# ueda0319/neddf

Hardware: NVIDIA H100
Metric: ray-samples/s (800x800x192) (higher is better)
Workload: dtype f16x3-split operands, f32 accumulate

## Files before the change

neddf_b200/csrc/field_tc.cu:

```cuda
#include "tc_ptx.cuh"

#include <algorithm>
#include <cstring>

namespace neddf {
namespace tc {

constexpr int kStages = 3;
constexpr int kConsumers = 256;
constexpr int kConsumerWarps = kConsumers / 32;
constexpr int kThreads = kConsumers + 128;
constexpr uint32_t kConsumerRegs = 232, kProducerRegs = 40;

constexpr uint32_t kOffHHi = 0;
constexpr uint32_t kOffHLo = kOffHHi + kHBytes;
constexpr uint32_t kOffAuxHi = kOffHLo + kHBytes;
constexpr uint32_t kOffAuxLo = kOffAuxHi + kAuxBytes;
constexpr uint32_t kOffRing = kOffAuxLo + kAuxBytes;
constexpr uint32_t kOffScratch = kOffRing + kStages * kChunkBytes;

struct Scratch {
  float geo[kTileS][12];
  uint64_t full[kStages];
  uint64_t empty[kStages];
};
constexpr uint32_t kSmemBytes = kOffScratch + sizeof(Scratch);
static_assert(kSmemBytes <= 227 * 1024, "shared memory budget");

constexpr int kGroup = kRows / kTileS;
constexpr uint32_t kParkH = kHBytes / kGroup, kParkAux = kAuxBytes / kGroup;
constexpr uint32_t kParkBytes = 2 * kParkH + 2 * kParkAux;

struct TcLayer {
  int aux_ksteps;
  int h_ksteps;
};

struct TcParams {
  FieldParams f;
  TcLayer layer[kMaxHidden];
  int chunks_per_tile;
  int dist_chunks;
  const unsigned char* w_tc;
  const float* bias;
  int* status;
  int eval;
  int density_only;
  unsigned char* park;
};

__device__ __forceinline__ uint32_t cluster_ctarank() {
  uint32_t r;
  asm volatile("mov.u32 %0, %%cluster_ctarank;" : "=r"(r));
  return r;
}
__device__ __forceinline__ void cluster_sync_all() {
  asm volatile("barrier.cluster.arrive.release.aligned;\nbarrier.cluster.wait.acquire.aligned;" ::: "memory");
}
__device__ __forceinline__ uint32_t mapa_u32(uint32_t saddr, uint32_t rank) {
  uint32_t r;
  asm volatile("mapa.shared::cluster.u32 %0, %1, %2;" : "=r"(r) : "r"(saddr), "r"(rank));
  return r;
}
__device__ __forceinline__ void mbar_arrive_remote(uint32_t caddr) {
  asm volatile("mbarrier.arrive.release.cluster.shared::cluster.b64 _, [%0];" ::"r"(caddr) : "memory");
}
__device__ __forceinline__ void mbar_wait_cluster(uint64_t* bar, uint32_t parity) {
  asm volatile(
      "{\n"
      ".reg .pred p;\n"
      "TC_WAITC:\n"
      "mbarrier.try_wait.parity.acquire.cluster.shared::cta.b64 p, [%0], %1;\n"
      "@p bra TC_DONEC;\n"
      "bra TC_WAITC;\n"
      "TC_DONEC:\n"
      "}\n" ::"r"(smem_u32(bar)),
      "r"(parity)
      : "memory");
}
__device__ __forceinline__ void tma_bulk_g2s_pair(uint32_t dst_smem, const void* src, uint32_t bytes, uint64_t* bar) {
  asm volatile(
      "cp.async.bulk.shared::cluster.global.mbarrier::complete_tx::bytes.multicast::cluster [%0], [%1], %2, [%3], %4;" ::"r"(
          dst_smem),
      "l"(src), "r"(bytes), "r"(smem_u32(bar)), "h"((uint16_t)3)
      : "memory");
}

__device__ __forceinline__ void tile_geometry(const FieldParams& p, float (*geo)[12], int64_t n0, int s, int64_t n_total) {
  const SampleIn in = sample_input(p, n0 + s, n_total);
#pragma unroll
  for (int i = 0; i < 3; ++i) {
    geo[s][i] = in.pos[i];
    geo[s][3 + i] = in.dir[i];
    geo[s][6 + i] = in.var[i];
  }
}

__device__ __forceinline__ void write_pos_embedding(const FieldParams& p, const float (*geo)[12], unsigned char* aux_hi,
                                                    unsigned char* aux_lo, int s, int sub, int nsub, bool scaled,
                                                    float& bad, int rows = 4) {
  const int half = 3 * p.embed_pos;
  for (int idx = sub; idx < half; idx += nsub) {
    int e = idx / 3, d = idx - 3 * e;
    PeEntry q = pe_entry(e, geo[s][d], geo[s][6 + d], p.lowpass[e]);
    float sc_ = scaled ? q.scale_s : q.scale_0;
    float g = q.freq * sc_;
    const float js = g * q.c, jc = -g * q.s;
    store_sample(aux_hi, aux_lo, kAuxK, s, idx, sc_ * q.s, d == 0 ? js : 0.f, d == 1 ? js : 0.f, d == 2 ? js : 0.f, bad, rows);
    store_sample(aux_hi, aux_lo, kAuxK, s, half + idx, sc_ * q.c, d == 0 ? jc : 0.f, d == 1 ? jc : 0.f, d == 2 ? jc : 0.f, bad, rows);
  }
}

__device__ __forceinline__ void bar_consumers() { asm volatile("bar.sync 1, %0;" ::"n"(kConsumers) : "memory"); }

template <bool kLoad>
__device__ __forceinline__ void park_move(unsigned char* smem, unsigned char* slot, int j, int tid) {
#pragma unroll
  for (int b = 0; b < 4; ++b) {
    const uint32_t bytes = b < 2 ? kParkH : kParkAux;
    const uint32_t so = (b == 0 ? kOffHHi : b == 1 ? kOffHLo : b == 2 ? kOffAuxHi : kOffAuxLo) + (uint32_t)j * bytes;
    const uint32_t go = b < 2 ? b * kParkH : 2 * kParkH + (b - 2) * kParkAux;
    uint4* s = reinterpret_cast<uint4*>(smem + so);
    uint4* g = slot ? reinterpret_cast<uint4*>(slot + go) : nullptr;
    constexpr int kIt = kParkH / 16 / kConsumers;
    uint4 v[kIt];
#pragma unroll
    for (int it = 0; it < kIt; ++it) {
      const uint32_t idx = tid + it * kConsumers;
      if (idx < bytes / 16) v[it] = kLoad ? (g ? g[idx] : make_uint4(0u, 0u, 0u, 0u)) : s[idx];
    }
#pragma unroll
    for (int it = 0; it < kIt; ++it) {
      const uint32_t idx = tid + it * kConsumers;
      if (idx < bytes / 16) {
        if (kLoad) s[idx] = v[it];
        else g[idx] = v[it];
      }
    }
  }
}

enum { kPhPrologue, kPhDistance, kPhHeads, kPhColour, kPhPark, kPhTiles, kPhCount };
#ifdef NEDDF_TC_PHASE_CLOCKS
__device__ unsigned long long g_tc_phase[kPhCount];
#define TC_PHASE(i)                        \
  do {                                     \
    if (tid == 0) {                        \
      const long long now_ = clock64();    \
      ph_sum[i] += now_ - ph_t;            \
      ph_t = now_;                         \
    }                                      \
  } while (0)
#else
#define TC_PHASE(i) \
  do {              \
  } while (0)
#endif

template <int ACT, bool PAIR>
__global__ void __launch_bounds__(kThreads, 1) field_tc_kernel(const __grid_constant__ TcParams P) {
  extern __shared__ __align__(1024) unsigned char smem[];
  const FieldParams& p = P.f;
  unsigned char* h_hi = smem + kOffHHi;
  unsigned char* h_lo = smem + kOffHLo;
  unsigned char* aux_hi = smem + kOffAuxHi;
  unsigned char* aux_lo = smem + kOffAuxLo;
  unsigned char* ring = smem + kOffRing;
  Scratch* sc = reinterpret_cast<Scratch*>(smem + kOffScratch);

  const int tid = threadIdx.x;
  const int warp = tid >> 5, lane = tid & 31;
  const int n_hidden = p.n_ddf + p.n_col;

  const int64_t n_total = field_total(p);
  const int64_t n_tiles = (n_total + kTileS - 1) / kTileS;
  const uint32_t rank = PAIR ? cluster_ctarank() : 0;
  const int64_t unit = PAIR ? (int64_t)(blockIdx.x >> 1) : (int64_t)blockIdx.x;
  const int64_t n_units = PAIR ? (int64_t)(gridDim.x >> 1) : (int64_t)gridDim.x;
  const int64_t units_total = PAIR ? (n_tiles + 1) / 2 : n_tiles;
  int64_t my_tiles = 0;
  if (unit < units_total) my_tiles = (units_total - 1 - unit) / n_units + 1;
  auto tile_of = [&](int64_t t) { return PAIR ? 2 * (unit + t * n_units) + rank : unit + t * n_units; };
  const int group = P.eval && !P.density_only ? kGroup : 1;
  const int chunks_end = P.density_only ? P.dist_chunks : P.chunks_per_tile;

  if (tid == 0) {
    for (int i = 0; i < kStages; ++i) {
      mbar_init(&sc->full[i], 1);
      mbar_init(&sc->empty[i], PAIR ? 2 * kConsumerWarps : kConsumerWarps);
    }
    mbar_fence_init();
  }
  __syncthreads();
  if (PAIR) cluster_sync_all();

  if (warp >= kConsumerWarps) {
    asm volatile("setmaxnreg.dec.sync.aligned.u32 %0;" ::"n"(kProducerRegs));
    if (warp == kConsumerWarps && lane == 0) {
      int64_t g = 0;
      auto push = [&](int c) {
        const int s = (int)(g % kStages);
        if (g >= kStages) mbar_wait_cluster(&sc->empty[s], (uint32_t)((g / kStages - 1) & 1));
        mbar_expect_tx(&sc->full[s], kChunkBytes);
        const unsigned char* src = P.w_tc + (size_t)c * kChunkBytes;
        const uint32_t dst = smem_u32(ring + s * kChunkBytes);
        if (PAIR) tma_bulk_g2s_pair(dst + rank * (kChunkBytes / 2), src + rank * (kChunkBytes / 2), kChunkBytes / 2, &sc->full[s]);
        else tma_bulk_g2s(dst, src, kChunkBytes, &sc->full[s]);
        ++g;
      };
      for (int64_t base = 0; base < my_tiles; base += group) {
        const int gn = (int)std::min<int64_t>(group, my_tiles - base);
        for (int i = 0; i < gn; ++i)
          for (int c = 0; c < P.dist_chunks; ++c) push(c);
        for (int c = P.dist_chunks; c < chunks_end; ++c) push(c);
      }
    }
  } else {
    asm volatile("setmaxnreg.inc.sync.aligned.u32 %0;" ::"n"(kConsumerRegs));
    const int wg = tid >> 7;
    const int chb = 128 * wg + 16 * ((tid & 127) >> 5) + (lane >> 2);
    const int cq = 2 * (lane & 3);
    const int hs = tid >> 3, hj = (tid >> 1) & 3, hk = tid & 1;
    const int hbase = lane & ~7;
    float bad = 0.f;
    __half2 badh = __floats2half2_rn(0.f, 0.f);
    uint32_t peer_empty[kStages];
#pragma unroll
    for (int i = 0; i < kStages; ++i) peer_empty[i] = PAIR ? mapa_u32(smem_u32(&sc->empty[i]), rank ^ 1) : 0u;
    auto release = [&](int64_t g) {
      if (lane == 0) {
        const int s = (int)(g % kStages);
        mbar_arrive(&sc->empty[s]);
        if (PAIR) mbar_arrive_remote(peer_empty[s]);
      }
    };
    int64_t g = 0;
    HeadOut head;
    std::memset(&head, 0, sizeof(head));
#ifdef NEDDF_TC_PHASE_CLOCKS
    long long ph_sum[kPhCount] = {}, ph_t = clock64();
#endif

    unsigned char* park = P.park + (size_t)blockIdx.x * kGroup * kParkBytes;

    auto layer = [&](int l, int64_t base, int gn) {
      const int64_t n0 = tile_of(base) * kTileS;
      const TcLayer L = P.layer[l];
      const bool cgroup = P.eval && l >= p.n_ddf;
      float acc[2][64];
#pragma unroll
      for (int i = 0; i < 64; ++i) {
        acc[0][i] = 0.f;
        acc[1][i] = 0.f;
      }
      fence_regs(acc[0]);
      fence_regs(acc[1]);
      const int nk = L.aux_ksteps + L.h_ksteps;
      for (int ks = 0; ks < nk; ++ks, ++g) {
        const int s = (int)(g % kStages);
        mbar_wait(&sc->full[s], (uint32_t)((g / kStages) & 1));
        const uint32_t w = smem_u32(ring + s * kChunkBytes);
        uint64_t bhi, blo;
        if (ks < L.aux_ksteps) {
          bhi = make_desc(smem_u32(aux_hi) + ks * 256, 128, kAuxK * 16);
          blo = make_desc(smem_u32(aux_lo) + ks * 256, 128, kAuxK * 16);
        } else {
          const int kh = ks - L.aux_ksteps;
          bhi = make_desc(smem_u32(h_hi) + kh * 256, 128, kHK * 16);
          blo = make_desc(smem_u32(h_lo) + kh * 256, 128, kHK * 16);
        }
        wgmma_fence();
#pragma unroll
        for (int mb = 0; mb < 2; ++mb) {
          const uint32_t aoff = (uint32_t)(16 * wg + 8 * mb) * 256;
          const uint64_t ahi = make_desc(w + aoff, 128, 256), alo = make_desc(w + kChunkBytes / 2 + aoff, 128, 256);
          wgmma_n128<0, 1>(acc[mb], ahi, bhi, 1);
          wgmma_n128<0, 1>(acc[mb], alo, bhi, 1);
          wgmma_n128<0, 1>(acc[mb], ahi, blo, 1);
        }
        wgmma_commit();
        if (ks > 0) {
          wgmma_wait<1>();
          release(g - 1);
        }
      }
      wgmma_wait<0>();
      fence_regs(acc[0]);
      fence_regs(acc[1]);
      release(g - 1);
      bar_consumers();

      const float* bias = P.bias + (size_t)l * kWidth;
#pragma unroll
      for (int mb = 0; mb < 2; ++mb) {
#pragma unroll
        for (int r = 0; r < 2; ++r) {
          const int ch = chb + 64 * mb + 8 * r;
          const float b = __ldg(bias + ch);
#pragma unroll
          for (int q = 0; q < 4; ++q) {
            float y[2], d1[2];
            const uint32_t off = (uint32_t)(q * (kHK * 16) + ch * 16 + cq * 2);
#pragma unroll
            for (int e = 0; e < 2; ++e) {
              const float xpre = acc[mb][4 * q + 2 * r + e] + b;
              if (p.save_pre) {
                const int64_t n = n0 + 8 * q + cq + e;
                if (n < n_total) {
                  float* dst = p.save_pre + (((size_t)l * p.n + n) * 4) * kWidth + ch;
                  dst[0] = xpre;
#pragma unroll
                  for (int j = 1; j < 4; ++j) dst[j * kWidth] = acc[mb][16 * j + 4 * q + 2 * r + e];
                }
              }
              tc_hidden_act<ACT>(xpre, y[e], d1[e]);
            }
            uint32_t hi, lo;
            split2h(y[0], y[1], hi, lo, badh);
            *reinterpret_cast<uint32_t*>(h_hi + off) = hi;
            *reinterpret_cast<uint32_t*>(h_lo + off) = lo;
            if (cgroup) {
#pragma unroll
              for (int j = 1; j < 4; ++j) {
#pragma unroll
                for (int e = 0; e < 2; ++e) tc_hidden_act<ACT>(acc[mb][16 * j + 4 * q + 2 * r + e] + b, y[e], d1[e]);
                split2h(y[0], y[1], hi, lo, badh);
                *reinterpret_cast<uint32_t*>(h_hi + off + j * 4 * (kHK * 16)) = hi;
                *reinterpret_cast<uint32_t*>(h_lo + off + j * 4 * (kHK * 16)) = lo;
              }
            } else {
#pragma unroll
              for (int j = 1; j < 4; ++j) {
                const float g0 = d1[0] * acc[mb][16 * j + 4 * q + 2 * r];
                const float g1 = d1[1] * acc[mb][16 * j + 4 * q + 2 * r + 1];
                split2h(g0, g1, hi, lo, badh);
                *reinterpret_cast<uint32_t*>(h_hi + off + j * 4 * (kHK * 16)) = hi;
                *reinterpret_cast<uint32_t*>(h_lo + off + j * 4 * (kHK * 16)) = lo;
              }
            }
          }
        }
      }
      bar_consumers();
      TC_PHASE(l < p.n_ddf ? kPhDistance : kPhColour);

      const int hrow = 32 * hj + hs;
      const uint32_t hrow_off = (uint32_t)((hrow >> 3) * (kHK * 16) + (hrow & 7) * 2);
      const int rot = hj + 4 * hk;
      auto hval = [&](int k) {
        return __half2float(*reinterpret_cast<const __half*>(h_hi + hrow_off + k * 16)) +
               __half2float(*reinterpret_cast<const __half*>(h_lo + hrow_off + k * 16));
      };
      if (l == p.n_ddf - 1) {
        float pd = 0.f, pa = 0.f;
#pragma unroll 4
        for (int kk = 0; kk < 128; ++kk) {
          const int k = 128 * hk + ((kk + rot) & 127);
          const float v = hval(k);
          const float2 wv = __ldg(reinterpret_cast<const float2*>(p.w_head_da) + k);
          pd = fmaf(v, wv.x, pd);
          pa = fmaf(v, wv.y, pa);
        }
        pd += __shfl_xor_sync(0xffffffffu, pd, 1);
        pa += __shfl_xor_sync(0xffffffffu, pa, 1);
        float ddf[4], aux[4];
#pragma unroll
        for (int j = 0; j < 4; ++j) {
          ddf[j] = __shfl_sync(0xffffffffu, pd, hbase + 2 * j);
          aux[j] = __shfl_sync(0xffffffffu, pa, hbase + 2 * j);
        }
        const int rows = P.eval ? 1 : 4;
        if (hj == 0 && hk == 0) {
          ddf[0] += __ldg(p.b_head + 0);
          aux[0] += __ldg(p.b_head + 1);
          head_density(ddf, aux, p.d_near, p.aux_grad_scale, p.density_act, head);
          const int kn = p.n_e0 + p.n_d;
          if (!P.density_only) {
#pragma unroll
            for (int c = 0; c < 3; ++c) store_sample(aux_hi, aux_lo, kAuxK, hs, kn + c, head.normal[c], 0.f, 0.f, 0.f, bad, rows);
          }
          const int64_t n = n0 + hs;
          if (n < n_total) {
            int64_t ray_, on;
            int j_;
            field_map(p, n, ray_, j_, on);
            if (p.distance) p.distance[on] = head.distance;
            if (p.density) p.density[on] = head.density;
            if (p.aux_grad) p.aux_grad[on] = head.aux;
          }
        }
        if (!P.density_only) {
          const int s = tid >> 3, sub = tid & 7;
          write_pos_embedding(p, sc->geo, aux_hi, aux_lo, s, sub, 8, false, bad, rows);
          const int dhalf = 3 * p.embed_dir;
          for (int idx = sub; idx < dhalf; idx += 8) {
            int e = idx / 3, d = idx - 3 * e;
            float sn, cs;
            sincosf((float)(1u << e) * sc->geo[s][3 + d], &sn, &cs);
            store_sample(aux_hi, aux_lo, kAuxK, s, p.n_e0 + idx, sn, 0.f, 0.f, 0.f, bad, rows);
            store_sample(aux_hi, aux_lo, kAuxK, s, p.n_e0 + dhalf + idx, cs, 0.f, 0.f, 0.f, bad, rows);
          }
          for (int k = p.n_e0 + p.n_d + 3 + sub; k < kAuxK; k += 8)
            store_sample(aux_hi, aux_lo, kAuxK, s, k, 0.f, 0.f, 0.f, 0.f, bad, rows);
        }
        bar_consumers();
      } else if (l == n_hidden - 1) {
        if (cgroup) {
          const int row = tid >> 1, ck = tid & 1;
          const uint32_t row_off = (uint32_t)((row >> 3) * (kHK * 16) + (row & 7) * 2);
          float pc[3] = {0.f, 0.f, 0.f};
#pragma unroll 4
          for (int kk = 0; kk < 128; ++kk) {
            const int k = 128 * ck + ((kk + 4 * ck) & 127);
            const float v = __half2float(*reinterpret_cast<const __half*>(h_hi + row_off + k * 16)) +
                            __half2float(*reinterpret_cast<const __half*>(h_lo + row_off + k * 16));
            const float4 wv = __ldg(reinterpret_cast<const float4*>(p.w_head_col) + k);
            pc[0] = fmaf(v, wv.x, pc[0]);
            pc[1] = fmaf(v, wv.y, pc[1]);
            pc[2] = fmaf(v, wv.z, pc[2]);
          }
#pragma unroll
          for (int c = 0; c < 3; ++c) pc[c] += __shfl_xor_sync(0xffffffffu, pc[c], 1);
          const int64_t n = tile_of(base + (row >> 5)) * kTileS + (row & 31);
          if (ck == 0 && (row >> 5) < gn && n < n_total && p.color) {
            int64_t ray_, on;
            int j_;
            field_map(p, n, ray_, j_, on);
#pragma unroll
            for (int c = 0; c < 3; ++c) p.color[3 * on + c] = pc[c] + __ldg(p.b_head + 2 + c);
          }
        } else {
          float pc[3] = {0.f, 0.f, 0.f};
#pragma unroll 4
          for (int kk = 0; kk < 128; ++kk) {
            const int k = 128 * hk + ((kk + rot) & 127);
            const float v = hval(k);
            const float4 wv = __ldg(reinterpret_cast<const float4*>(p.w_head_col) + k);
            pc[0] = fmaf(v, wv.x, pc[0]);
            pc[1] = fmaf(v, wv.y, pc[1]);
            pc[2] = fmaf(v, wv.z, pc[2]);
          }
          float colv[4][3];
#pragma unroll
          for (int c = 0; c < 3; ++c) {
            pc[c] += __shfl_xor_sync(0xffffffffu, pc[c], 1);
#pragma unroll
            for (int j = 0; j < 4; ++j) colv[j][c] = __shfl_sync(0xffffffffu, pc[c], hbase + 2 * j);
          }
          const int64_t n = n0 + hs;
          if (hj == 0 && hk == 0 && n < n_total) {
            float col[3], colJ[3][3];
#pragma unroll
            for (int c = 0; c < 3; ++c) {
              col[c] = colv[0][c] + __ldg(p.b_head + 2 + c);
#pragma unroll
              for (int j = 0; j < 3; ++j) colJ[j][c] = colv[1 + j][c];
            }
            int64_t ray_, on;
            int j_;
            field_map(p, n, ray_, j_, on);
            if (p.color) {
              p.color[3 * on + 0] = col[0];
              p.color[3 * on + 1] = col[1];
              p.color[3 * on + 2] = col[2];
            }
            if (p.penalty) p.penalty[on] = field_penalty(head, col, colJ, p.distance_range_max, p.penalty_weight);
          }
        }
      }
      fence_async_smem();
      bar_consumers();
      TC_PHASE(l == p.n_ddf - 1 || l == n_hidden - 1 ? kPhHeads : l < p.n_ddf ? kPhDistance : kPhColour);
    };

    for (int64_t base = 0; base < my_tiles; base += group) {
      const int gn = (int)std::min<int64_t>(group, my_tiles - base);
      for (int gi = 0; gi < gn; ++gi) {
        const int64_t n0 = tile_of(base + gi) * kTileS;
        if (tid < kTileS) tile_geometry(p, sc->geo, n0, tid, n_total);
        bar_consumers();
        {
          const int s = tid >> 3, sub = tid & 7;
          write_pos_embedding(p, sc->geo, aux_hi, aux_lo, s, sub, 8, true, bad);
          for (int k = p.n_e0 + sub; k < 64; k += 8) store_sample(aux_hi, aux_lo, kAuxK, s, k, 0.f, 0.f, 0.f, 0.f, bad);
        }
        fence_async_smem();
        bar_consumers();
        TC_PHASE(kPhPrologue);
#ifdef NEDDF_TC_PHASE_CLOCKS
        if (tid == 0) ++ph_sum[kPhTiles];
#endif
        for (int l = 0; l < p.n_ddf; ++l) layer(l, base + gi, 1);
        if (P.eval && !P.density_only) {
          park_move<false>(smem, park + gi * kParkBytes, 0, tid);
          TC_PHASE(kPhPark);
        }
      }
      if (P.density_only) continue;
      if (P.eval) {
        bar_consumers();
        for (int j = 0; j < kGroup; ++j) park_move<true>(smem, j < gn ? park + j * kParkBytes : nullptr, j, tid);
        fence_async_smem();
        bar_consumers();
        TC_PHASE(kPhPark);
      }
      for (int l = p.n_ddf; l < n_hidden; ++l) layer(l, base, gn);
    }
#ifdef NEDDF_TC_PHASE_CLOCKS
    if (tid == 0)
      for (int i = 0; i < kPhCount; ++i) atomicAdd(&g_tc_phase[i], (unsigned long long)ph_sum[i]);
#endif
    const float2 m = __half22float2(badh);
    if (!(fmaxf(bad, fmaxf(m.x, m.y)) < 65504.0f) && P.status) atomicOr(P.status, 4);
  }
  if (PAIR) cluster_sync_all();
}

struct TcPackArgs {
  const float* w[kMaxHidden];
  const float* b[kMaxHidden];
  int k_in[kMaxHidden];
  int aux_real[kMaxHidden];
  int aux_pad[kMaxHidden];
  int ksteps[kMaxHidden];
  int chunk0[kMaxHidden];
  int n_hidden;
};

__global__ void tc_pack_hidden_kernel(TcPackArgs a, unsigned char* __restrict__ dst, float* __restrict__ bias) {
  const int l = blockIdx.y;
  const int total = a.ksteps[l] * kWidth * 16;
  for (int idx = blockIdx.x * blockDim.x + threadIdx.x; idx < total; idx += gridDim.x * blockDim.x) {
    const int k = idx & 15, m = (idx >> 4) & (kWidth - 1), ks = idx >> 12;
    const int kk = ks * 16 + k;
    int row;
    if (kk < a.aux_pad[l]) row = (kk < a.aux_real[l]) ? kk : -1;
    else row = a.aux_real[l] + (kk - a.aux_pad[l]);
    if (row >= a.k_in[l]) row = -1;
    const float w = (row >= 0) ? a.w[l][(size_t)row * kWidth + m] : 0.f;
    const __half hi = __float2half_rn(w);
    const __half lo = __float2half_rn(w - __half2float(hi));
    unsigned char* chunk = dst + (size_t)(a.chunk0[l] + ks) * kChunkBytes;
    *reinterpret_cast<__half*>(chunk + wchunk_off(m, k)) = hi;
    *reinterpret_cast<__half*>(chunk + kChunkBytes / 2 + wchunk_off(m, k)) = lo;
  }
  if (blockIdx.x == 0)
    for (int c = threadIdx.x; c < kWidth; c += blockDim.x) bias[l * kWidth + c] = a.b[l][c];
}

struct TcStorage {
  unsigned char* d_w = nullptr;
  float* d_bias = nullptr;
  int* d_status = nullptr;
  unsigned char* d_park = nullptr;
  int chunks_per_tile = 0;
  int dist_chunks = 0;
  TcLayer layer[kMaxHidden];
  TcPackArgs pack;
};

template <int N>
__global__ void __launch_bounds__(256, 1) tc_selftest_kernel(const float* __restrict__ A, const float* __restrict__ B, int k,
                                                            float* __restrict__ C) {
  extern __shared__ __align__(1024) unsigned char smem[];
  constexpr int kA = kChunkBytes / 2;
  const int ksteps = k / 16;
  unsigned char* a_buf = smem;
  unsigned char* b_hi = smem + (size_t)ksteps * kA;
  unsigned char* b_lo = b_hi + (size_t)N * k * 2;
  const int tid = threadIdx.x;
  for (int i = tid; i < 128 * k; i += blockDim.x) {
    const int m = i / k, kk = i % k;
    const float v = A[i];
    const __half hi = __float2half_rn(v), lo = __float2half_rn(v - __half2float(hi));
    unsigned char* chunk = a_buf + (size_t)(kk / 16) * kA;
    *reinterpret_cast<__half*>(chunk + wchunk_off(m, kk & 15)) = hi;
    *reinterpret_cast<__half*>(chunk + kA / 2 + wchunk_off(m, kk & 15)) = lo;
  }
  for (int i = tid; i < N * k; i += blockDim.x) {
    const int n = i / k, kk = i % k;
    const float v = B[i];
    const __half hi = __float2half_rn(v), lo = __float2half_rn(v - __half2float(hi));
    *reinterpret_cast<__half*>(b_hi + act_off(n, kk, k)) = hi;
    *reinterpret_cast<__half*>(b_lo + act_off(n, kk, k)) = lo;
  }
  fence_async_smem();
  __syncthreads();
  if (tid < 128 * 2) {
    const int wg = tid >> 7, lane = tid & 31;
    constexpr int R = N / 2;
    float acc[R];
#pragma unroll
    for (int i = 0; i < R; ++i) acc[i] = 0.f;
    fence_regs(acc);
    wgmma_fence();
    for (int ks = 0; ks < ksteps; ++ks) {
      const uint32_t w = smem_u32(a_buf + (size_t)ks * kA) + (uint32_t)(8 * wg) * 256;
      const uint64_t ahi = make_desc(w, 128, 256), alo = make_desc(w + kA / 2, 128, 256);
      const uint64_t bhi = make_desc(smem_u32(b_hi) + ks * 256, 128, k * 16), blo = make_desc(smem_u32(b_lo) + ks * 256, 128, k * 16);
      if constexpr (N == 128) {
        wgmma_n128<0, 1>(acc, ahi, bhi, 1);
        wgmma_n128<0, 1>(acc, alo, bhi, 1);
        wgmma_n128<0, 1>(acc, ahi, blo, 1);
      } else {
        wgmma_n16<0, 1>(acc, ahi, bhi, 1);
        wgmma_n16<0, 1>(acc, alo, bhi, 1);
        wgmma_n16<0, 1>(acc, ahi, blo, 1);
      }
    }
    wgmma_commit();
    wgmma_wait<0>();
    fence_regs(acc);
    const int row = 64 * wg + 16 * ((tid & 127) >> 5) + (lane >> 2);
#pragma unroll
    for (int i = 0; i < R; ++i) {
      const int m = row + 8 * ((i >> 1) & 1), n = 8 * (i >> 2) + 2 * (lane & 3) + (i & 1);
      C[(size_t)m * N + n] = acc[i];
    }
  }
}

}

static bool is_skip_layer(const neddf_field* f, int l) {
  for (int i = 0; i < f->cfg.n_skips; ++i)
    if (f->cfg.skips[i] == l - 1) return true;
  return false;
}

bool tc_supported(const neddf_field* f) {
  const int n_e0 = 6 * f->cfg.embed_pos_rank, off_h = n_e0 + 6 * f->cfg.embed_dir_rank + 3;
  return n_e0 <= 64 && off_h <= tc::kAuxK && f->cfg.ddf_layer_width == kWidth && f->cfg.col_layer_width == kWidth;
}

static int32_t tc_ensure(neddf_field* f) {
  if (f->tc) return NEDDF_OK;
  tc::TcStorage* S = new tc::TcStorage();
  const int n_hidden = f->n_ddf + f->n_col;
  int chunk = 0;
  std::memset(&S->pack, 0, sizeof(S->pack));
  S->pack.n_hidden = n_hidden;
  for (int l = 0; l < n_hidden; ++l) {
    int aux_real = 0, aux_pad = 0, h_k = 0;
    if (l == 0) { aux_real = f->proto.n_e0; aux_pad = 64; }
    else if (l < f->n_ddf) { if (is_skip_layer(f, l)) { aux_real = f->proto.n_e0; aux_pad = 64; } h_k = kWidth; }
    else if (l == f->n_ddf) { aux_real = f->proto.off_h; aux_pad = tc::kAuxK; h_k = kWidth; }
    else h_k = kWidth;
    S->layer[l].aux_ksteps = aux_pad / 16;
    S->layer[l].h_ksteps = h_k / 16;
    S->pack.k_in[l] = f->shape_in[l];
    S->pack.aux_real[l] = aux_real;
    S->pack.aux_pad[l] = aux_pad;
    S->pack.ksteps[l] = S->layer[l].aux_ksteps + S->layer[l].h_ksteps;
    S->pack.chunk0[l] = chunk;
    chunk += S->pack.ksteps[l];
    if (l == f->n_ddf - 1) S->dist_chunks = chunk;
  }
  S->chunks_per_tile = chunk;
  if (cudaMalloc(&S->d_w, (size_t)chunk * tc::kChunkBytes) != cudaSuccess ||
      cudaMalloc(&S->d_bias, (size_t)n_hidden * kWidth * sizeof(float)) != cudaSuccess ||
      cudaMalloc(&S->d_status, sizeof(int)) != cudaSuccess) {
    cudaFree(S->d_w); cudaFree(S->d_bias); cudaFree(S->d_status);
    delete S;
    return fail(NEDDF_E_CUDA, "tensor-core engine: cudaMalloc failed");
  }
  cudaMemset(S->d_status, 0, sizeof(int));
  f->tc = S;
  return NEDDF_OK;
}

void tc_destroy(neddf_field* f) {
  if (!f->tc) return;
  tc::TcStorage* S = static_cast<tc::TcStorage*>(f->tc);
  cudaFree(S->d_w);
  cudaFree(S->d_bias);
  cudaFree(S->d_status);
  cudaFree(S->d_park);
  delete S;
  f->tc = nullptr;
}

int32_t tc_pack_weights(neddf_field* f, const float* const* d_w, const float* const* d_b, cudaStream_t s) {
  int32_t rc = tc_ensure(f);
  if (rc != NEDDF_OK) return rc;
  tc::TcStorage* S = static_cast<tc::TcStorage*>(f->tc);
  tc::TcPackArgs a = S->pack;
  const int n_hidden = f->n_ddf + f->n_col;
  for (int l = 0; l < n_hidden; ++l) {
    a.w[l] = d_w[l];
    a.b[l] = d_b[l];
  }
  tc::tc_pack_hidden_kernel<<<dim3(64, n_hidden), 256, 0, s>>>(a, S->d_w, S->d_bias);
  NEDDF_LAUNCH_CHECK();
  return NEDDF_OK;
}

int32_t launch_field_tc(const neddf_field* f, FieldParams& p, int flags, bool pair, cudaStream_t s) {
  tc::TcStorage* S = static_cast<tc::TcStorage*>(f->tc);
  if (!S) return fail(NEDDF_E_INVALID, "tensor-core engine: weights were never packed");
  tc::TcParams P;
  P.f = p;
  for (int l = 0; l < p.n_ddf + p.n_col; ++l) P.layer[l] = S->layer[l];
  P.chunks_per_tile = S->chunks_per_tile;
  P.dist_chunks = S->dist_chunks;
  P.w_tc = S->d_w;
  P.bias = S->d_bias;
  P.status = S->d_status;
  P.eval = (flags == NEDDF_OUT_EVAL && p.penalty == nullptr && p.save_pre == nullptr) ? 1 : 0;
  P.density_only = (p.color == nullptr && p.penalty == nullptr && p.save_pre == nullptr) ? 1 : 0;
  if (P.eval && !P.density_only && !S->d_park) {
    if (cudaMalloc(&S->d_park, (size_t)sm_count() * tc::kGroup * tc::kParkBytes) != cudaSuccess) {
      S->d_park = nullptr;
      return fail(NEDDF_E_CUDA, "tensor-core engine: cudaMalloc of the colour-trunk scratch failed");
    }
  }
  P.park = S->d_park;
  const int64_t n_tiles = (p.n + tc::kTileS - 1) / tc::kTileS;
  auto launch = [&](auto kern) -> int32_t {
    NEDDF_CUDA_CHECK(cudaFuncSetAttribute(kern, cudaFuncAttributeMaxDynamicSharedMemorySize, (int)tc::kSmemBytes));
    cudaLaunchConfig_t cfg = {};
    cudaLaunchAttribute attr[1];
    cfg.blockDim = dim3(tc::kThreads);
    cfg.dynamicSmemBytes = tc::kSmemBytes;
    cfg.stream = s;
    if (pair) {
      const int64_t pairs = (n_tiles + 1) / 2;
      cfg.gridDim = dim3((unsigned)(2 * std::max<int64_t>(1, std::min<int64_t>(pairs, sm_count() / 2))));
      attr[0].id = cudaLaunchAttributeClusterDimension;
      attr[0].val.clusterDim.x = 2;
      attr[0].val.clusterDim.y = 1;
      attr[0].val.clusterDim.z = 1;
      cfg.attrs = attr;
      cfg.numAttrs = 1;
    } else {
      cfg.gridDim = dim3((unsigned)std::max<int64_t>(1, std::min<int64_t>(n_tiles, sm_count())));
      cfg.numAttrs = 0;
    }
    NEDDF_CUDA_CHECK(cudaLaunchKernelEx(&cfg, kern, P));
    NEDDF_LAUNCH_CHECK();
    return NEDDF_OK;
  };
  switch (p.hidden_act) {
    case NEDDF_ACT_TANHEXP: return pair ? launch(tc::field_tc_kernel<NEDDF_ACT_TANHEXP, true>) : launch(tc::field_tc_kernel<NEDDF_ACT_TANHEXP, false>);
    case NEDDF_ACT_RELU: return pair ? launch(tc::field_tc_kernel<NEDDF_ACT_RELU, true>) : launch(tc::field_tc_kernel<NEDDF_ACT_RELU, false>);
    case NEDDF_ACT_LEAKYRELU: return pair ? launch(tc::field_tc_kernel<NEDDF_ACT_LEAKYRELU, true>) : launch(tc::field_tc_kernel<NEDDF_ACT_LEAKYRELU, false>);
  }
  return fail(NEDDF_E_INVALID, "tensor-core engine: unknown activation");
}

int32_t tc_read_status(const neddf_field* f, int* out, cudaStream_t s) {
  tc::TcStorage* S = static_cast<tc::TcStorage*>(f->tc);
  *out = 0;
  if (!S) return NEDDF_OK;
  NEDDF_CUDA_CHECK(cudaMemcpyAsync(out, S->d_status, sizeof(int), cudaMemcpyDeviceToHost, s));
  NEDDF_CUDA_CHECK(cudaStreamSynchronize(s));
  NEDDF_CUDA_CHECK(cudaMemsetAsync(S->d_status, 0, sizeof(int), s));
  return NEDDF_OK;
}

}

extern "C" int32_t neddf_tc_selftest(const float* d_a, const float* d_b, int32_t m, int32_t n, int32_t k, float* d_c,
                                     void* stream) {
  using namespace neddf;
  if (m != 128 || (n != 128 && n != 16) || k < 16 || (k % 16) != 0 || k > (n == 128 ? 128 : 256))
    return fail(NEDDF_E_INVALID, "neddf_tc_selftest: need m=128, n in {128,16}, k multiple of 16 (<=128 for n=128, <=256 for n=16)");
  if (!d_a || !d_b || !d_c) return fail(NEDDF_E_INVALID, "neddf_tc_selftest: NULL pointer");
  const size_t smem = (size_t)(k / 16) * (tc::kChunkBytes / 2) + (size_t)2 * n * k * 2;
  auto launch = [&](auto kern) -> int32_t {
    NEDDF_CUDA_CHECK(cudaFuncSetAttribute(kern, cudaFuncAttributeMaxDynamicSharedMemorySize, (int)smem));
    kern<<<1, 256, smem, (cudaStream_t)stream>>>(d_a, d_b, k, d_c);
    NEDDF_LAUNCH_CHECK();
    return NEDDF_OK;
  };
  return n == 128 ? launch(tc::tc_selftest_kernel<128>) : launch(tc::tc_selftest_kernel<16>);
// ... 13 lines not shown
```

neddf_b200/csrc/tc_ptx.cuh:

```cuda
#pragma once

#include "field_math.cuh"
#include "mbarrier.cuh"

#include <cuda_fp16.h>

namespace neddf {
namespace tc {

constexpr int kTileS = 32;
constexpr int kRows = 4 * kTileS;
constexpr int kHK = 256;
constexpr int kAuxK = 96;
constexpr int kChunkBytes = 16384;
constexpr uint32_t kHBytes = kRows * kHK * 2;
constexpr uint32_t kAuxBytes = kRows * kAuxK * 2;

__host__ __device__ __forceinline__ uint32_t act_off(int row, int k, int KC) {
  return (uint32_t)((row >> 3) * (KC * 16) + k * 16 + (row & 7) * 2);
}
__host__ __device__ __forceinline__ uint32_t wchunk_off(int m, int k) {
  return (uint32_t)((m >> 3) * 256 + (k >> 3) * 128 + (m & 7) * 16 + (k & 7) * 2);
}

__device__ __forceinline__ void fence_async_smem() { asm volatile("fence.proxy.async.shared::cta;" ::: "memory"); }

__device__ __forceinline__ uint64_t make_desc(uint32_t saddr, uint32_t lbo_bytes, uint32_t sbo_bytes) {
  uint64_t d = 0;
  d |= (uint64_t)((saddr >> 4) & 0x3FFFu);
  d |= (uint64_t)((lbo_bytes >> 4) & 0x3FFFu) << 16;
  d |= (uint64_t)((sbo_bytes >> 4) & 0x3FFFu) << 32;
  return d;
}

__device__ __forceinline__ void wgmma_fence() { asm volatile("wgmma.fence.sync.aligned;" ::: "memory"); }
__device__ __forceinline__ void wgmma_commit() { asm volatile("wgmma.commit_group.sync.aligned;" ::: "memory"); }
template <int N>
__device__ __forceinline__ void wgmma_wait() {
  asm volatile("wgmma.wait_group.sync.aligned %0;" ::"n"(N) : "memory");
}
template <int R>
__device__ __forceinline__ void fence_regs(float (&d)[R]) {
#pragma unroll
  for (int i = 0; i < R; ++i) asm volatile("" : "+f"(d[i])::"memory");
}

template <int TA, int TB>
__device__ __forceinline__ void wgmma_n16(float (&d)[8], uint64_t a, uint64_t b, uint32_t acc) {
  asm volatile(
      "{\n.reg .pred p;\nsetp.ne.b32 p, %10, 0;\n"
      "wgmma.mma_async.sync.aligned.m64n16k16.f32.f16.f16 {%0,%1,%2,%3,%4,%5,%6,%7}, %8, %9, p, 1, 1, %11, %12;\n}\n"
      : "+f"(d[0]), "+f"(d[1]), "+f"(d[2]), "+f"(d[3]), "+f"(d[4]), "+f"(d[5]), "+f"(d[6]), "+f"(d[7])
      : "l"(a), "l"(b), "r"(acc), "n"(TA), "n"(TB));
}
template <int TA, int TB>
__device__ __forceinline__ void wgmma_n128(float (&d)[64], uint64_t a, uint64_t b, uint32_t acc) {
  asm volatile(
      "{\n.reg .pred p;\nsetp.ne.b32 p, %66, 0;\n"
      "wgmma.mma_async.sync.aligned.m64n128k16.f32.f16.f16 {%0,%1,%2,%3,%4,%5,%6,%7,%8,%9,%10,%11,%12,%13,%14,%15,%16,%17,%18,"
      "%19,%20,%21,%22,%23,%24,%25,%26,%27,%28,%29,%30,%31,%32,%33,%34,%35,%36,%37,%38,%39,%40,%41,%42,%43,%44,%45,%46,%47,%48,"
      "%49,%50,%51,%52,%53,%54,%55,%56,%57,%58,%59,%60,%61,%62,%63}, %64, %65, p, 1, 1, %67, %68;\n}\n"
      : "+f"(d[0]), "+f"(d[1]), "+f"(d[2]), "+f"(d[3]), "+f"(d[4]), "+f"(d[5]), "+f"(d[6]), "+f"(d[7]), "+f"(d[8]), "+f"(d[9]),
        "+f"(d[10]), "+f"(d[11]), "+f"(d[12]), "+f"(d[13]), "+f"(d[14]), "+f"(d[15]), "+f"(d[16]), "+f"(d[17]), "+f"(d[18]),
        "+f"(d[19]), "+f"(d[20]), "+f"(d[21]), "+f"(d[22]), "+f"(d[23]), "+f"(d[24]), "+f"(d[25]), "+f"(d[26]), "+f"(d[27]),
        "+f"(d[28]), "+f"(d[29]), "+f"(d[30]), "+f"(d[31]), "+f"(d[32]), "+f"(d[33]), "+f"(d[34]), "+f"(d[35]), "+f"(d[36]),
        "+f"(d[37]), "+f"(d[38]), "+f"(d[39]), "+f"(d[40]), "+f"(d[41]), "+f"(d[42]), "+f"(d[43]), "+f"(d[44]), "+f"(d[45]),
        "+f"(d[46]), "+f"(d[47]), "+f"(d[48]), "+f"(d[49]), "+f"(d[50]), "+f"(d[51]), "+f"(d[52]), "+f"(d[53]), "+f"(d[54]),
        "+f"(d[55]), "+f"(d[56]), "+f"(d[57]), "+f"(d[58]), "+f"(d[59]), "+f"(d[60]), "+f"(d[61]), "+f"(d[62]), "+f"(d[63])
      : "l"(a), "l"(b), "r"(acc), "n"(TA), "n"(TB));
}

template <int TA, int TB>
__device__ __forceinline__ void wgmma_n256(float (&d)[128], uint64_t a, uint64_t b, uint32_t acc) {
  asm volatile(
      "{\n.reg .pred p;\nsetp.ne.b32 p, %130, 0;\n"
      "wgmma.mma_async.sync.aligned.m64n256k16.f32.f16.f16 {%0,%1,%2,%3,%4,%5,%6,%7,%8,%9,%10,%11,%12,%13,%14,%15,%16,%17,%18,%19,%20,%21,%22,%23,%24,%25,%26,%27,%28,%29,%30,%31,%32,%33,%34,%35,%36,%37,%38,%39,%40,%41,%42,%43,%44,%45,%46,%47,%48,%49,%50,%51,%52,%53,%54,%55,%56,%57,%58,%59,%60,%61,%62,%63,%64,%65,%66,%67,%68,%69,%70,%71,%72,%73,%74,%75,%76,%77,%78,%79,%80,%81,%82,%83,%84,%85,%86,%87,%88,%89,%90,%91,%92,%93,%94,%95,%96,%97,%98,%99,%100,%101,%102,%103,%104,%105,%106,%107,%108,%109,%110,%111,%112,%113,%114,%115,%116,%117,%118,%119,%120,%121,%122,%123,%124,%125,%126,%127}, %128, %129, p, 1, 1, %131, %132;\n}\n"
      : "+f"(d[0]), "+f"(d[1]), "+f"(d[2]), "+f"(d[3]), "+f"(d[4]), "+f"(d[5]), "+f"(d[6]), "+f"(d[7]), "+f"(d[8]), "+f"(d[9]), "+f"(d[10]), "+f"(d[11]), "+f"(d[12]), "+f"(d[13]), "+f"(d[14]), "+f"(d[15]), "+f"(d[16]), "+f"(d[17]), "+f"(d[18]), "+f"(d[19]), "+f"(d[20]), "+f"(d[21]), "+f"(d[22]), "+f"(d[23]), "+f"(d[24]), "+f"(d[25]), "+f"(d[26]), "+f"(d[27]), "+f"(d[28]), "+f"(d[29]), "+f"(d[30]), "+f"(d[31]), "+f"(d[32]), "+f"(d[33]), "+f"(d[34]), "+f"(d[35]), "+f"(d[36]), "+f"(d[37]), "+f"(d[38]), "+f"(d[39]), "+f"(d[40]), "+f"(d[41]), "+f"(d[42]), "+f"(d[43]), "+f"(d[44]), "+f"(d[45]), "+f"(d[46]), "+f"(d[47]), "+f"(d[48]), "+f"(d[49]), "+f"(d[50]), "+f"(d[51]), "+f"(d[52]), "+f"(d[53]), "+f"(d[54]), "+f"(d[55]), "+f"(d[56]), "+f"(d[57]), "+f"(d[58]), "+f"(d[59]), "+f"(d[60]), "+f"(d[61]), "+f"(d[62]), "+f"(d[63]), "+f"(d[64]), "+f"(d[65]), "+f"(d[66]), "+f"(d[67]), "+f"(d[68]), "+f"(d[69]), "+f"(d[70]), "+f"(d[71]), "+f"(d[72]), "+f"(d[73]), "+f"(d[74]), "+f"(d[75]), "+f"(d[76]), "+f"(d[77]), "+f"(d[78]), "+f"(d[79]), "+f"(d[80]), "+f"(d[81]), "+f"(d[82]), "+f"(d[83]), "+f"(d[84]), "+f"(d[85]), "+f"(d[86]), "+f"(d[87]), "+f"(d[88]), "+f"(d[89]), "+f"(d[90]), "+f"(d[91]), "+f"(d[92]), "+f"(d[93]), "+f"(d[94]), "+f"(d[95]), "+f"(d[96]), "+f"(d[97]), "+f"(d[98]), "+f"(d[99]), "+f"(d[100]), "+f"(d[101]), "+f"(d[102]), "+f"(d[103]), "+f"(d[104]), "+f"(d[105]), "+f"(d[106]), "+f"(d[107]), "+f"(d[108]), "+f"(d[109]), "+f"(d[110]), "+f"(d[111]), "+f"(d[112]), "+f"(d[113]), "+f"(d[114]), "+f"(d[115]), "+f"(d[116]), "+f"(d[117]), "+f"(d[118]), "+f"(d[119]), "+f"(d[120]), "+f"(d[121]), "+f"(d[122]), "+f"(d[123]), "+f"(d[124]), "+f"(d[125]), "+f"(d[126]), "+f"(d[127])
      : "l"(a), "l"(b), "r"(acc), "n"(TA), "n"(TB));
}

__device__ __forceinline__ float ex2_approx(float x) {
  float y;
  asm("ex2.approx.ftz.f32 %0, %1;" : "=f"(y) : "f"(x));
  return y;
}
__device__ __forceinline__ float rcp_approx(float x) {
  float y;
  asm("rcp.approx.ftz.f32 %0, %1;" : "=f"(y) : "f"(x));
  return y;
}

__device__ __forceinline__ void tanhexp_fast(float x, float& y, float& d1) {
  const float kL2E = 1.4426950408889634f, kL2E_lo = 1.9259629911266175e-8f, kLn2 = 0.6931471805599453f;
  float t = x * kL2E;
  float r = fmaf(x, kL2E, -t) + x * kL2E_lo;
  float ex = ex2_approx(t);
  ex = fmaf(ex, r * kLn2, ex);
  float E = ex2_approx(ex * (2.0f * kL2E));
  float tx_big = fmaf(-2.0f, rcp_approx(E + 1.0f), 1.0f);
  float u2 = ex * ex;
  float poly = fmaf(u2, fmaf(u2, fmaf(u2, -17.0f / 315.0f, 2.0f / 15.0f), -1.0f / 3.0f), 1.0f);
  float tx = (ex < 0.125f) ? ex * poly : tx_big;
  float yy = x * tx;
  float dd = tx - x * ex * (tx * tx - 1.0f);
  const bool big = x > 20.0f;
  y = big ? x : yy;
  d1 = big ? 1.0f : dd;
}

template <int ACT>
__device__ __forceinline__ void tc_hidden_act(float x, float& y, float& d1) {
  if (ACT == NEDDF_ACT_TANHEXP) tanhexp_fast(x, y, d1);
  else hidden_act<ACT>(x, y, d1);
}

__device__ __forceinline__ void split2(float a, float b, uint32_t& hi, uint32_t& lo, float& amax) {
  __half2 h = __floats2half2_rn(a, b);
  float2 hf = __half22float2(h);
  __half2 l = __floats2half2_rn(a - hf.x, b - hf.y);
  hi = *reinterpret_cast<uint32_t*>(&h);
  lo = *reinterpret_cast<uint32_t*>(&l);
  amax = fmaxf(amax, fmaxf(fabsf(a), fabsf(b)));
}

__device__ __forceinline__ void split2h(float a, float b, uint32_t& hi, uint32_t& lo, __half2& amax) {
  __half2 h = __floats2half2_rn(a, b);
  float2 hf = __half22float2(h);
  __half2 l = __floats2half2_rn(a - hf.x, b - hf.y);
  hi = *reinterpret_cast<uint32_t*>(&h);
  lo = *reinterpret_cast<uint32_t*>(&l);
  amax = __hmax2(amax, __habs2(h));
}

__device__ __forceinline__ void store_sample(unsigned char* hi_buf, unsigned char* lo_buf, int KC, int s, int k,
                                             float v0, float v1, float v2, float v3, float& bad, int rows = 4) {
// ... 20 lines not shown
```

Before: 30.99 million.

## Compute distance and colour heads with wgmma over packed head-weight chunks

Replaces the scalar per-thread dot-product heads (reading split-half activations from shared memory and weights via __ldg) with a wgmma m64n64k16 pass using a new packed 8-row head weight chunk streamed through the existing TMA ring. The positional/direction embedding writes now overlap the asynchronous head MMA, and results are staged through a shared head buffer. This adds two extra chunks per tile to the weight stream, an extra barrier, and recomputes head_density for the penalty path. It also adds range checking of packed weights.

```diff
diff --git a/neddf_b200/csrc/field_tc.cu b/neddf_b200/csrc/field_tc.cu
--- a/neddf_b200/csrc/field_tc.cu
+++ b/neddf_b200/csrc/field_tc.cu
@@ -20,7 +20,8 @@
 constexpr uint32_t kOffScratch = kOffRing + kStages * kChunkBytes;
 
 struct Scratch {
-  float geo[kTileS][12];
+  float geo[kTileS][9];
+  float head[3][kRows];
   uint64_t full[kStages];
   uint64_t empty[kStages];
 };
@@ -86,7 +87,7 @@
       : "memory");
 }
 
-__device__ __forceinline__ void tile_geometry(const FieldParams& p, float (*geo)[12], int64_t n0, int s, int64_t n_total) {
+__device__ __forceinline__ void tile_geometry(const FieldParams& p, float (*geo)[9], int64_t n0, int s, int64_t n_total) {
   const SampleIn in = sample_input(p, n0 + s, n_total);
 #pragma unroll
   for (int i = 0; i < 3; ++i) {
@@ -96,7 +97,7 @@
   }
 }
 
-__device__ __forceinline__ void write_pos_embedding(const FieldParams& p, const float (*geo)[12], unsigned char* aux_hi,
+__device__ __forceinline__ void write_pos_embedding(const FieldParams& p, const float (*geo)[9], unsigned char* aux_hi,
                                                     unsigned char* aux_lo, int s, int sub, int nsub, bool scaled,
                                                     float& bad, int rows = 4) {
   const int half = 3 * p.embed_pos;
@@ -220,23 +221,17 @@
     const int wg = tid >> 7;
     const int chb = 128 * wg + 16 * ((tid & 127) >> 5) + (lane >> 2);
     const int cq = 2 * (lane & 3);
-    const int hs = tid >> 3, hj = (tid >> 1) & 3, hk = tid & 1;
-    const int hbase = lane & ~7;
     float bad = 0.f;
     __half2 badh = __floats2half2_rn(0.f, 0.f);
-    uint32_t peer_empty[kStages];
-#pragma unroll
-    for (int i = 0; i < kStages; ++i) peer_empty[i] = PAIR ? mapa_u32(smem_u32(&sc->empty[i]), rank ^ 1) : 0u;
     auto release = [&](int64_t g) {
       if (lane == 0) {
         const int s = (int)(g % kStages);
         mbar_arrive(&sc->empty[s]);
-        if (PAIR) mbar_arrive_remote(peer_empty[s]);
+        if (PAIR) mbar_arrive_remote(mapa_u32(smem_u32(&sc->empty[s]), rank ^ 1));
       }
     };
     int64_t g = 0;
-    HeadOut head;
-    std::memset(&head, 0, sizeof(head));
+    float ddf[4] = {0.f, 0.f, 0.f, 0.f}, aux[4] = {0.f, 0.f, 0.f, 0.f};
 #ifdef NEDDF_TC_PHASE_CLOCKS
     long long ph_sum[kPhCount] = {}, ph_t = clock64();
 #endif
@@ -341,55 +336,48 @@
           }
         }
       }
+      const bool dist_head = l == p.n_ddf - 1, col_head = l == n_hidden - 1;
+      if (dist_head || col_head) fence_async_smem();
       bar_consumers();
       TC_PHASE(l < p.n_ddf ? kPhDistance : kPhColour);
 
-      const int hrow = 32 * hj + hs;
-      const uint32_t hrow_off = (uint32_t)((hrow >> 3) * (kHK * 16) + (hrow & 7) * 2);
-      const int rot = hj + 4 * hk;
-      auto hval = [&](int k) {
-        return __half2float(*reinterpret_cast<const __half*>(h_hi + hrow_off + k * 16)) +
-               __half2float(*reinterpret_cast<const __half*>(h_lo + hrow_off + k * 16));
+      auto head_mma = [&](auto&& overlap) {
+        float hacc[32];
+#pragma unroll
+        for (int i = 0; i < 32; ++i) hacc[i] = 0.f;
+        fence_regs(hacc);
+        const uint32_t bh = smem_u32(h_hi) + (uint32_t)wg * 8 * (kHK * 16), bl = smem_u32(h_lo) + (uint32_t)wg * 8 * (kHK * 16);
+        const int s = (int)(g % kStages);
+        mbar_wait(&sc->full[s], (uint32_t)((g / kStages) & 1));
+        const uint32_t w = smem_u32(ring + s * kChunkBytes);
+        wgmma_fence();
+#pragma unroll 1
+        for (int ks = 0; ks < kHK / 16; ++ks) {
+          const uint64_t ahi = make_desc(w + ks * 256, 128, 0), alo = make_desc(w + kChunkBytes / 2 + ks * 256, 128, 0);
+          const uint64_t bhi = make_desc(bh + ks * 256, 128, kHK * 16), blo = make_desc(bl + ks * 256, 128, kHK * 16);
+          wgmma_n64<0, 1>(hacc, ahi, bhi, 1);
+          wgmma_n64<0, 1>(hacc, alo, bhi, 1);
+          wgmma_n64<0, 1>(hacc, ahi, blo, 1);
+        }
+        wgmma_commit();
+        overlap();
+        wgmma_wait<0>();
+        fence_regs(hacc);
+        release(g);
+        ++g;
+        if ((tid & 127) < 12) {
+          const int m = lane >> 2;
+#pragma unroll
+          for (int i = 0; i < 32; ++i)
+            if (((i >> 1) & 1) == 0) sc->head[m][64 * wg + 8 * (i >> 2) + cq + (i & 1)] = hacc[i];
+        }
+        bar_consumers();
       };
-      if (l == p.n_ddf - 1) {
-        float pd = 0.f, pa = 0.f;
-#pragma unroll 4
-        for (int kk = 0; kk < 128; ++kk) {
-          const int k = 128 * hk + ((kk + rot) & 127);
-          const float v = hval(k);
-          const float2 wv = __ldg(reinterpret_cast<const float2*>(p.w_head_da) + k);
-          pd = fmaf(v, wv.x, pd);
-          pa = fmaf(v, wv.y, pa);
-        }
-        pd += __shfl_xor_sync(0xffffffffu, pd, 1);
-        pa += __shfl_xor_sync(0xffffffffu, pa, 1);
-        float ddf[4], aux[4];
-#pragma unroll
-        for (int j = 0; j < 4; ++j) {
-          ddf[j] = __shfl_sync(0xffffffffu, pd, hbase + 2 * j);
-          aux[j] = __shfl_sync(0xffffffffu, pa, hbase + 2 * j);
-        }
+
+      if (dist_head) {
         const int rows = P.eval ? 1 : 4;
-        if (hj == 0 && hk == 0) {
-          ddf[0] += __ldg(p.b_head + 0);
-          aux[0] += __ldg(p.b_head + 1);
-          head_density(ddf, aux, p.d_near, p.aux_grad_scale, p.density_act, head);
-          const int kn = p.n_e0 + p.n_d;
-          if (!P.density_only) {
-#pragma unroll
-            for (int c = 0; c < 3; ++c) store_sample(aux_hi, aux_lo, kAuxK, hs, kn + c, head.normal[c], 0.f, 0.f, 0.f, bad, rows);
-          }
-          const int64_t n = n0 + hs;
-          if (n < n_total) {
-            int64_t ray_, on;
-            int j_;
-            field_map(p, n, ray_, j_, on);
-            if (p.distance) p.distance[on] = head.distance;
-            if (p.density) p.density[on] = head.density;
-            if (p.aux_grad) p.aux_grad[on] = head.aux;
-          }
-        }
-        if (!P.density_only) {
+        head_mma([&] {
+          if (P.density_only) return;
           const int s = tid >> 3, sub = tid & 7;
           write_pos_embedding(p, sc->geo, aux_hi, aux_lo, s, sub, 8, false, bad, rows);
           const int dhalf = 3 * p.embed_dir;
@@ -402,59 +390,53 @@
           }
           for (int k = p.n_e0 + p.n_d + 3 + sub; k < kAuxK; k += 8)
             store_sample(aux_hi, aux_lo, kAuxK, s, k, 0.f, 0.f, 0.f, 0.f, bad, rows);
-        }
-        bar_consumers();
-      } else if (l == n_hidden - 1) {
-        if (cgroup) {
-          const int row = tid >> 1, ck = tid & 1;
-          const uint32_t row_off = (uint32_t)((row >> 3) * (kHK * 16) + (row & 7) * 2);
-          float pc[3] = {0.f, 0.f, 0.f};
-#pragma unroll 4
-          for (int kk = 0; kk < 128; ++kk) {
-            const int k = 128 * ck + ((kk + 4 * ck) & 127);
-            const float v = __half2float(*reinterpret_cast<const __half*>(h_hi + row_off + k * 16)) +
-                            __half2float(*reinterpret_cast<const __half*>(h_lo + row_off + k * 16));
-            const float4 wv = __ldg(reinterpret_cast<const float4*>(p.w_head_col) + k);
-            pc[0] = fmaf(v, wv.x, pc[0]);
-            pc[1] = fmaf(v, wv.y, pc[1]);
-            pc[2] = fmaf(v, wv.z, pc[2]);
+        });
+        if (tid < kTileS) {
+#pragma unroll
+          for (int j = 0; j < 4; ++j) {
+            ddf[j] = sc->head[0][32 * j + tid];
+            aux[j] = sc->head[1][32 * j + tid];
           }
-#pragma unroll
-          for (int c = 0; c < 3; ++c) pc[c] += __shfl_xor_sync(0xffffffffu, pc[c], 1);
-          const int64_t n = tile_of(base + (row >> 5)) * kTileS + (row & 31);
-          if (ck == 0 && (row >> 5) < gn && n < n_total && p.color) {
+          ddf[0] += __ldg(p.b_head + 0);
+          aux[0] += __ldg(p.b_head + 1);
+          HeadOut head;
+          head_density(ddf, aux, p.d_near, p.aux_grad_scale, p.density_act, head);
+          const int kn = p.n_e0 + p.n_d;
+          if (!P.density_only) {
+#pragma unroll
+            for (int c = 0; c < 3; ++c) store_sample(aux_hi, aux_lo, kAuxK, tid, kn + c, head.normal[c], 0.f, 0.f, 0.f, bad, rows);
+          }
+          const int64_t n = n0 + tid;
+          if (n < n_total) {
             int64_t ray_, on;
             int j_;
             field_map(p, n, ray_, j_, on);
-#pragma unroll
-            for (int c = 0; c < 3; ++c) p.color[3 * on + c] = pc[c] + __ldg(p.b_head + 2 + c);
+            if (p.distance) p.distance[on] = head.distance;
+            if (p.density) p.density[on] = head.density;
+            if (p.aux_grad) p.aux_grad[on] = head.aux;
+          }
+        }
+      } else if (col_head) {
+        head_mma([] {});
+        if (cgroup) {
+          const int row = tid;
+          const int64_t n = tile_of(base + (row >> 5)) * kTileS + (row & 31);
+          if (row < kRows && (row >> 5) < gn && n < n_total && p.color) {
+            int64_t ray_, on;
+            int j_;
+            field_map(p, n, ray_, j_, on);
+#pragma unroll
+            for (int c = 0; c < 3; ++c) p.color[3 * on + c] = sc->head[c][row] + __ldg(p.b_head + 2 + c);
           }
         } else {
-          float pc[3] = {0.f, 0.f, 0.f};
-#pragma unroll 4
-          for (int kk = 0; kk < 128; ++kk) {
-            const int k = 128 * hk + ((kk + rot) & 127);
-            const float v = hval(k);
-            const float4 wv = __ldg(reinterpret_cast<const float4*>(p.w_head_col) + k);
-            pc[0] = fmaf(v, wv.x, pc[0]);
-            pc[1] = fmaf(v, wv.y, pc[1]);
-            pc[2] = fmaf(v, wv.z, pc[2]);
-          }
-          float colv[4][3];
-#pragma unroll
-          for (int c = 0; c < 3; ++c) {
-            pc[c] += __shfl_xor_sync(0xffffffffu, pc[c], 1);
-#pragma unroll
-            for (int j = 0; j < 4; ++j) colv[j][c] = __shfl_sync(0xffffffffu, pc[c], hbase + 2 * j);
-          }
-          const int64_t n = n0 + hs;
-          if (hj == 0 && hk == 0 && n < n_total) {
+          const int64_t n = n0 + tid;
+          if (tid < kTileS && n < n_total) {
             float col[3], colJ[3][3];
 #pragma unroll
             for (int c = 0; c < 3; ++c) {
-              col[c] = colv[0][c] + __ldg(p.b_head + 2 + c);
-#pragma unroll
-              for (int j = 0; j < 3; ++j) colJ[j][c] = colv[1 + j][c];
+              col[c] = sc->head[c][tid] + __ldg(p.b_head + 2 + c);
+#pragma unroll
+              for (int j = 0; j < 3; ++j) colJ[j][c] = sc->head[c][32 * (1 + j) + tid];
             }
             int64_t ray_, on;
             int j_;
@@ -464,7 +446,11 @@
               p.color[3 * on + 1] = col[1];
               p.color[3 * on + 2] = col[2];
             }
-            if (p.penalty) p.penalty[on] = field_penalty(head, col, colJ, p.distance_range_max, p.penalty_weight);
+            if (p.penalty) {
+              HeadOut head;
+              head_density(ddf, aux, p.d_near, p.aux_grad_scale, p.density_act, head);
+              p.penalty[on] = field_penalty(head, col, colJ, p.distance_range_max, p.penalty_weight);
+            }
           }
         }
       }
@@ -511,7 +497,7 @@
       for (int i = 0; i < kPhCount; ++i) atomicAdd(&g_tc_phase[i], (unsigned long long)ph_sum[i]);
 #endif
     const float2 m = __half22float2(badh);
-    if (!(fmaxf(bad, fmaxf(m.x, m.y)) < 65504.0f) && P.status) atomicOr(P.status, 4);
+    if (P.status && (!(fmaxf(bad, fmaxf(m.x, m.y)) < 65504.0f) || P.status[1])) atomicOr(P.status, 4);
   }
   if (PAIR) cluster_sync_all();
 }
@@ -527,7 +513,7 @@
   int n_hidden;
 };
 
-__global__ void tc_pack_hidden_kernel(TcPackArgs a, unsigned char* __restrict__ dst, float* __restrict__ bias) {
+__global__ void tc_pack_hidden_kernel(TcPackArgs a, unsigned char* __restrict__ dst, float* __restrict__ bias, int* wrange) {
   const int l = blockIdx.y;
   const int total = a.ksteps[l] * kWidth * 16;
   for (int idx = blockIdx.x * blockDim.x + threadIdx.x; idx < total; idx += gridDim.x * blockDim.x) {
@@ -538,6 +524,7 @@
     else row = a.aux_real[l] + (kk - a.aux_pad[l]);
     if (row >= a.k_in[l]) row = -1;
     const float w = (row >= 0) ? a.w[l][(size_t)row * kWidth + m] : 0.f;
+    if (fabsf(w) >= 65504.0f) *wrange = 1;
     const __half hi = __float2half_rn(w);
     const __half lo = __float2half_rn(w - __half2float(hi));
     unsigned char* chunk = dst + (size_t)(a.chunk0[l] + ks) * kChunkBytes;
@@ -546,6 +533,23 @@
   }
   if (blockIdx.x == 0)
     for (int c = threadIdx.x; c < kWidth; c += blockDim.x) bias[l * kWidth + c] = a.b[l][c];
+}
+
+__global__ void tc_pack_heads_kernel(const float* w_ddf, const float* w_aux, const float* w_col, int chunk0_da,
+                                     int chunk0_col, unsigned char* __restrict__ dst, int* wrange) {
+  const bool colour = blockIdx.x == 1;
+  for (int idx = threadIdx.x; idx < kHeadRows * kWidth; idx += blockDim.x) {
+    const int m = idx / kWidth, k = idx - m * kWidth;
+    float w = 0.f;
+    if (colour && m < 3) w = w_col[3 * k + m];
+    else if (!colour && m < 2) w = (m == 0 ? w_ddf : w_aux)[k];
+    if (fabsf(w) >= 65504.0f) *wrange = 1;
+    const __half hi = __float2half_rn(w);
+    const __half lo = __float2half_rn(w - __half2float(hi));
+    unsigned char* chunk = dst + (size_t)(colour ? chunk0_col : chunk0_da) * kChunkBytes;
+    *reinterpret_cast<__half*>(chunk + hchunk_off(m, k)) = hi;
+    *reinterpret_cast<__half*>(chunk + kChunkBytes / 2 + hchunk_off(m, k)) = lo;
+  }
 }
 
 struct TcStorage {
@@ -555,6 +559,7 @@
   unsigned char* d_park = nullptr;
   int chunks_per_tile = 0;
   int dist_chunks = 0;
+  int head_chunk0[2] = {0, 0};
   TcLayer layer[kMaxHidden];
   TcPackArgs pack;
 };
@@ -654,17 +659,23 @@
     S->pack.ksteps[l] = S->layer[l].aux_ksteps + S->layer[l].h_ksteps;
     S->pack.chunk0[l] = chunk;
     chunk += S->pack.ksteps[l];
-    if (l == f->n_ddf - 1) S->dist_chunks = chunk;
-  }
+    if (l == f->n_ddf - 1) {
+      S->head_chunk0[0] = chunk;
+      chunk += 1;
+      S->dist_chunks = chunk;
+    }
+  }
+  S->head_chunk0[1] = chunk;
+  chunk += 1;
   S->chunks_per_tile = chunk;
   if (cudaMalloc(&S->d_w, (size_t)chunk * tc::kChunkBytes) != cudaSuccess ||
       cudaMalloc(&S->d_bias, (size_t)n_hidden * kWidth * sizeof(float)) != cudaSuccess ||
-      cudaMalloc(&S->d_status, sizeof(int)) != cudaSuccess) {
+      cudaMalloc(&S->d_status, 2 * sizeof(int)) != cudaSuccess) {
     cudaFree(S->d_w); cudaFree(S->d_bias); cudaFree(S->d_status);
     delete S;
     return fail(NEDDF_E_CUDA, "tensor-core engine: cudaMalloc failed");
   }
-  cudaMemset(S->d_status, 0, sizeof(int));
+  cudaMemset(S->d_status, 0, 2 * sizeof(int));
   f->tc = S;
   return NEDDF_OK;
 }
@@ -690,7 +701,11 @@
     a.w[l] = d_w[l];
     a.b[l] = d_b[l];
   }
-  tc::tc_pack_hidden_kernel<<<dim3(64, n_hidden), 256, 0, s>>>(a, S->d_w, S->d_bias);
+  NEDDF_CUDA_CHECK(cudaMemsetAsync(S->d_status + 1, 0, sizeof(int), s));
+  tc::tc_pack_hidden_kernel<<<dim3(64, n_hidden), 256, 0, s>>>(a, S->d_w, S->d_bias, S->d_status + 1);
+  NEDDF_LAUNCH_CHECK();
+  tc::tc_pack_heads_kernel<<<2, 256, 0, s>>>(d_w[n_hidden], d_w[n_hidden + 1], d_w[n_hidden + 2], S->head_chunk0[0],
+                                             S->head_chunk0[1], S->d_w, S->d_status + 1);
   NEDDF_LAUNCH_CHECK();
   return NEDDF_OK;
 }
diff --git a/neddf_b200/csrc/tc_ptx.cuh b/neddf_b200/csrc/tc_ptx.cuh
--- a/neddf_b200/csrc/tc_ptx.cuh
+++ b/neddf_b200/csrc/tc_ptx.cuh
@@ -13,6 +13,7 @@
 constexpr int kHK = 256;
 constexpr int kAuxK = 96;
 constexpr int kChunkBytes = 16384;
+constexpr int kHeadRows = 8;
 constexpr uint32_t kHBytes = kRows * kHK * 2;
 constexpr uint32_t kAuxBytes = kRows * kAuxK * 2;
 
@@ -21,6 +22,9 @@
 }
 __host__ __device__ __forceinline__ uint32_t wchunk_off(int m, int k) {
   return (uint32_t)((m >> 3) * 256 + (k >> 3) * 128 + (m & 7) * 16 + (k & 7) * 2);
+}
+__host__ __device__ __forceinline__ uint32_t hchunk_off(int m, int k) {
+  return (uint32_t)((k >> 4) * 256 + wchunk_off(m, k & 15));
 }
 
 __device__ __forceinline__ void fence_async_smem() { asm volatile("fence.proxy.async.shared::cta;" ::: "memory"); }
@@ -51,6 +55,18 @@
       "{\n.reg .pred p;\nsetp.ne.b32 p, %10, 0;\n"
       "wgmma.mma_async.sync.aligned.m64n16k16.f32.f16.f16 {%0,%1,%2,%3,%4,%5,%6,%7}, %8, %9, p, 1, 1, %11, %12;\n}\n"
       : "+f"(d[0]), "+f"(d[1]), "+f"(d[2]), "+f"(d[3]), "+f"(d[4]), "+f"(d[5]), "+f"(d[6]), "+f"(d[7])
+      : "l"(a), "l"(b), "r"(acc), "n"(TA), "n"(TB));
+}
+template <int TA, int TB>
+__device__ __forceinline__ void wgmma_n64(float (&d)[32], uint64_t a, uint64_t b, uint32_t acc) {
+  asm volatile(
+      "{\n.reg .pred p;\nsetp.ne.b32 p, %34, 0;\n"
+      "wgmma.mma_async.sync.aligned.m64n64k16.f32.f16.f16 {%0,%1,%2,%3,%4,%5,%6,%7,%8,%9,%10,%11,%12,%13,%14,%15,%16,%17,%18,"
+      "%19,%20,%21,%22,%23,%24,%25,%26,%27,%28,%29,%30,%31}, %32, %33, p, 1, 1, %35, %36;\n}\n"
+      : "+f"(d[0]), "+f"(d[1]), "+f"(d[2]), "+f"(d[3]), "+f"(d[4]), "+f"(d[5]), "+f"(d[6]), "+f"(d[7]), "+f"(d[8]), "+f"(d[9]),
+        "+f"(d[10]), "+f"(d[11]), "+f"(d[12]), "+f"(d[13]), "+f"(d[14]), "+f"(d[15]), "+f"(d[16]), "+f"(d[17]), "+f"(d[18]),
+        "+f"(d[19]), "+f"(d[20]), "+f"(d[21]), "+f"(d[22]), "+f"(d[23]), "+f"(d[24]), "+f"(d[25]), "+f"(d[26]), "+f"(d[27]),
+        "+f"(d[28]), "+f"(d[29]), "+f"(d[30]), "+f"(d[31])
       : "l"(a), "l"(b), "r"(acc), "n"(TA), "n"(TB));
 }
 template <int TA, int TB>
```

After: 32.05 million, median of 6. +3.4%, better.
